# KMASAHIRO/AVR

Hardware: AMD Instinct MI355X
Metric: ray-samples/sec/GPU (1024 rays×256 samp×512 freq) + IR render ms/pose (higher is better)
Workload: dtype f32; 1 GPU; c2_meshrir_1024x256x512; mode=pose, rays=1024, samples=256, T=1022, freq_bins=512, distinct_poses=16, parallelism=poses x1 (no data-path collective)

## Files before the change

### avr_amd/_lib.py

```python
from __future__ import annotations

import ctypes
import math
import os
import threading

import numpy as np
import torch

_HERE = os.path.dirname(os.path.abspath(__file__))
LIB_PATH = os.path.join(_HERE, "libavr_hip.so")

DTYPE_F32 = 0
DTYPE_F16 = 1
DTYPE_BF16 = 2
MAX_AZI = 512
IRFFT_MAX_N = 13476

_c_i32 = ctypes.c_int32
_c_i64 = ctypes.c_int64
_c_f32 = ctypes.c_float
_vp = ctypes.c_void_p


class RenderParams(ctypes.Structure):

    _fields_ = [
        ("n_azi", _c_i32),
        ("n_ele", _c_i32),
        ("n_samples", _c_i32),
        ("T", _c_i32),
        ("n_rays", _c_i32),
        ("depth_scale", _c_f32),
        ("depth_offset", _c_f32),
        ("lo", _c_f32),
        ("span", _c_f32),
        ("fs", _c_f32),
        ("speed", _c_f32),
# ... 22 lines not shown
    p.n_ele = int(cfg["n_ele"])
    p.n_samples = int(cfg["n_samples"])
    p.T = int(T)
    p.n_rays = p.n_azi * p.n_ele + 2 if n_rays is None else int(n_rays)
    p.depth_scale = _f32(cfg["far"] - cfg["near"])
    p.depth_offset = _f32(cfg["near"])
    p.lo = _f32(cfg["xyz_min"])
    p.span = _f32(cfg["xyz_max"] - cfg["xyz_min"])
    p.fs = _f32(cfg["fs"])
    p.speed = _f32(cfg["speed"])
    p.pathloss = _f32(cfg["pathloss"])
    p.azi_jitter = _f32(np.pi * 2 / cfg["n_azi"])
    p.two_pi = _f32(np.pi * 2)
    p.phase_c = _f32((-2 * np.pi) / T)
    p.near_clamp = int(0.1 / cfg["speed"] * cfg["fs"])
    p.pl_len = int(math.ceil(T * 2.5))
    return p


class TablePtrs(ctypes.Structure):

    _fields_ = [("d_vals", ctypes.c_void_p), ("shift", ctypes.c_void_p),
                ("pl_table", ctypes.c_void_p), ("phase", ctypes.c_void_p),
                ("twiddle", ctypes.c_void_p), ("ir_twiddle", ctypes.c_void_p)]


_SIGS = {
    "avr_last_error": (ctypes.c_char_p, []),
    "avr_abi_version": (ctypes.c_int, []),
    "avr_pinned_alloc": (ctypes.c_int, [_c_i64, _vp, _vp]),
    "avr_pinned_free": (ctypes.c_int, [_vp]),
    "avr_graph_launch": (ctypes.c_int, [_vp, _vp]),
    "avr_tables": (ctypes.c_int, [_vp, _vp, _vp, _vp, _vp, _vp, _vp, _vp]),
    "avr_depth_samples": (ctypes.c_int, [_vp, _vp, _vp]),
    "avr_ir_twiddle": (ctypes.c_int, [_c_i32, _vp, _vp]),
    "avr_ray_directions": (ctypes.c_int, [_vp, _vp, _vp, _vp]),
    "avr_sample_points": (ctypes.c_int, [_vp, _c_i32] + [_vp] * 10),
    "avr_sample_rays": (ctypes.c_int, [_vp, _c_i32, _vp, _c_i32] + [_vp] * 9),
    "avr_weights_fwd": (ctypes.c_int, [_vp, _c_i32, _vp, _c_i32] + [_vp] * 7),
    "avr_ray_reduce_fwd": (ctypes.c_int, [_vp, _c_i32, _vp, _c_i32, _vp, _vp, _c_i32, _vp, _vp]),
    "avr_sample_rays_dev": (ctypes.c_int, [_vp, _c_i32, _vp, _c_i32] + [_vp] * 9),
    "avr_sample_rays_staged": (ctypes.c_int, [_vp, _c_i32, _vp, _c_i32, _c_i32] + [_vp] * 7),
    "avr_reduce_splits": (ctypes.c_int, [_vp, _c_i32, _c_i32, _vp]),
    "avr_dft_phase_fwd": (ctypes.c_int, [_vp, _c_i32, _vp, _c_i32, _vp, _vp, _vp, _vp, _c_i32, _vp, _vp]),
    "avr_spectrum_finalize": (ctypes.c_int, [_c_i32, _c_i32, _c_i32, _vp, _vp, _vp]),
    "avr_irfft": (ctypes.c_int, [_c_i32, _c_i32, _vp, _vp, _vp, _vp]),
    "avr_irfft_bwd": (ctypes.c_int, [_c_i32, _c_i32, _vp, _vp, _vp, _vp]),
    "avr_dft_phase_bwd": (ctypes.c_int, [_vp, _c_i32] + [_vp] * 7),
    "avr_ray_reduce_bwd": (ctypes.c_int, [_vp, _c_i32, _vp, _c_i32] + [_vp] * 6),
    "avr_weights_bwd": (ctypes.c_int, [_vp, _c_i32, _vp, _c_i32, _vp, _vp, _vp, _vp]),
    "avr_hashgrid_fwd": (ctypes.c_int, [_c_i64, _c_i32, _vp, _vp, _c_i32, _vp, _vp, _vp, _vp, _c_i32, _vp]),
    "avr_hashgrid_fwd_lm": (ctypes.c_int, [_c_i64, _c_i32, _vp, _vp, _c_i32, _vp, _vp, _vp, _vp, _c_i32, _vp]),
    "avr_hashgrid_fwd_lm_unit": (ctypes.c_int, [_c_i64, _c_i32, _vp, _vp, _c_i32, _vp, _vp, _vp, _vp, _c_i32, _vp]),
    "avr_ray_pose_bias": (ctypes.c_int, [_c_i32, _c_i32, _c_i32, _vp, _vp, _c_i32, _vp, _vp, _vp, _vp,
                                         _c_i32, _vp, _vp, _vp, _vp, _c_i32, _c_i32, _c_i32, _vp, _vp,
                                         _c_i32, _vp, _vp]),
    "avr_hashgrid_bwd": (ctypes.c_int, [_c_i64, _c_i32, _vp, _vp, _c_i32, _vp, _vp, _vp, _vp, _vp]),
    "avr_hashgrid_bwd_workspace": (ctypes.c_int, [_c_i64, _c_i32, _vp, _vp]),
    "avr_hashgrid_bwd_partitioned": (ctypes.c_int, [_c_i64, _c_i32, _vp, _vp, _c_i32, _vp, _vp, _vp, _vp, _vp,
                                                    _c_i64, _vp]),
    "avr_hashgrid_bwd_partitioned_set": (ctypes.c_int, [_c_i64, _c_i32, _vp, _vp, _c_i32, _vp, _vp, _vp, _vp, _vp,
                                                    _c_i64, _vp]),
    "avr_linear_wgrad_splits": (ctypes.c_int, [_c_i64, _c_i32, _c_i32, _vp]),
    "avr_linear512_pack_w2": (ctypes.c_int, [_vp, _c_i32, _c_i32, _vp, _vp]),
    "avr_linear512_mask_fwd": (ctypes.c_int, [_c_i64, _vp, _vp, _c_i32, _vp, _vp, _vp]),
    "avr_linear_wgrad": (ctypes.c_int, [_c_i64, _c_i32, _c_i32, _vp, _vp, _vp, _c_i32, _vp, _vp]),
    "avr_linear_out1_fwd": (ctypes.c_int, [_c_i64, _c_i32, _vp, _vp, _c_i32, _vp, _vp]),
    "avr_narrow_mm": (ctypes.c_int, [_c_i64, _c_i32, _c_i32, _vp, _vp, _c_i32, _c_i32, _vp, _vp, _vp]),
# ... 112 lines not shown
```

### avr_amd/csrc/render_fwd.hip

```cpp
#include "common.h"

#include <cstdlib>

using namespace avr;

typedef float floatx16 __attribute__((ext_vector_type(16)));

namespace {

constexpr double kTwoPi = 6.283185307179586476925286766559;

__global__ void tables_kernel(avr_render_params p, float* __restrict__ d_vals,
                              float* __restrict__ frac, int32_t* __restrict__ shift,
                              float* __restrict__ pl, float2* __restrict__ phase,
                              float2* __restrict__ tw) {
    const int S = p.n_samples, T = p.T, F = T / 2 + 1;
    const int64_t gid = (int64_t)blockIdx.x * blockDim.x + threadIdx.x;
    const int64_t stride = (int64_t)gridDim.x * blockDim.x;
    for (int64_t i = gid; i < S; i += stride) {
        const float d = linspace_at(0.0f, 1.0f, S, (int)i) * p.depth_scale + p.depth_offset;
        const float fr = (p.fs * d) / p.speed;
        d_vals[i] = d;
        frac[i] = fr;
        shift[i] = (int32_t)rintf(fr);
// ... 517 lines not shown
    const float2* src = spart + (int64_t)b * P * F + fc;
    float ax = 0.f, ay = 0.f;
    for (int q0 = 0; q0 < P; q0 += 64) {
        float2 v[4];
#pragma unroll
        for (int u = 0; u < 4; ++u) v[u] = src[(int64_t)min(q0 + g + 16 * u, P - 1) * F];
#pragma unroll
        for (int u = 0; u < 4; ++u)
            if (q0 + g + 16 * u < P) {
                ax += v[u].x;
                ay += v[u].y;
            }
    }
    red[g][j] = make_float2(ax, ay);
    __syncthreads();
    if (g == 0 && f < F) {
        float2 r = red[0][j];
        for (int k = 1; k < 16; ++k) {
            r.x += red[k][j].x;
            r.y += red[k][j].y;
        }
        out[(int64_t)b * F + f] = r;
    }
}

constexpr int kIrfftRedRows = 8;
constexpr size_t irfft_lds(int n) { return (size_t)(n / 2 + 1 + n) * sizeof(float2); }
constexpr size_t irfft_bwd_lds(int n) { return (size_t)n * (sizeof(float2) + sizeof(float)); }
constexpr size_t kIrfftStatic = kIrfftRedRows * 33 * sizeof(float);
constexpr size_t kIrfftBwdStatic = kIrfftRedRows * 33 * sizeof(float2);
static_assert(irfft_lds(kIrfftMaxN) + kIrfftStatic <= kLdsPerCu &&
                  irfft_bwd_lds(kIrfftMaxN) + kIrfftBwdStatic <= kLdsPerCu,
              "AVR_IRFFT_MAX_N must launch in both transforms");
static_assert(kIrfftMaxN % 2 == 0 && irfft_bwd_lds(kIrfftMaxN + 2) + kIrfftBwdStatic > kLdsPerCu,
              "AVR_IRFFT_MAX_N is the largest even length that launches in both");

__global__ __launch_bounds__(256) void irfft_kernel(int F, int B1, const float2* __restrict__ spec,
                                                    const float2* __restrict__ spec2,
                                                    const float2* __restrict__ twg,
                                                    float* __restrict__ ir, float* __restrict__ ir2) {
    extern __shared__ float2 lds[];
    __shared__ float red[kIrfftRedRows][33];
    const int n = 2 * (F - 1);
    float2* X = lds;
    float2* tw = lds + F;
    int b = blockIdx.y;
// ... 349 lines not shown
        return launch("avr_dft_phase_fwd", kern, grid, dim3(kDftThreads), lds, as_stream(stream), *p, part,
                      pl_table, shift, reinterpret_cast<const float2*>(phase),
                      reinterpret_cast<const float2*>(twiddle), reinterpret_cast<float2*>(spart), (int)B, S, T,
                      (int)k_split, kchunk, xcd_order);
    };
    switch (n_split) {
        case 1: return go(dft_phase_fwd_kernel<1>);
        case 2: return go(dft_phase_fwd_kernel<2>);
        case 4: return go(dft_phase_fwd_kernel<4>);
        case 8: return go(dft_phase_fwd_kernel<8>);
        case 16: return go(dft_phase_fwd_kernel<16>);
    }
    return fail(AVR_E_ARG, "avr_dft_phase_fwd: n_split must be 1, 2, 4, 8 or 16");
}

extern "C" int avr_spectrum_finalize(int32_t B, int32_t P, int32_t F, const float* spart,
                                     float* out, void* stream) {
    AVR_REQUIRE(B >= 1 && P >= 1 && F >= 1 && spart && out, "avr_spectrum_finalize: bad args");
    return launch("avr_spectrum_finalize", spectrum_finalize_kernel, dim3((unsigned)((F + 15) / 16), B), dim3(256),
                  0, as_stream(stream), (int)B, (int)P, (int)F, reinterpret_cast<const float2*>(spart),
                  reinterpret_cast<float2*>(out));
}

namespace avr {
int launch_irfft(int B, int F, const float* spec, const float* spec2, const float* tw, float* ir,
                 float* ir2, void* stream) {
    AVR_REQUIRE(B >= 1 && F >= 2 && spec && tw && ir, "avr_irfft: bad args");
    const int n = 2 * (F - 1);
    AVR_REQUIRE(n <= kIrfftMaxN, "avr_irfft: " AVR_IRFFT_LIMIT_TEXT);
    const size_t lds = irfft_lds(n);
    const int rows = spec2 ? 2 * B : B;
    return launch("avr_irfft", irfft_kernel, dim3((n + 31) / 32, rows), dim3(256), lds, as_stream(stream),
                  (int)F, (int)B, reinterpret_cast<const float2*>(spec),
                  reinterpret_cast<const float2*>(spec2 ? spec2 : spec), reinterpret_cast<const float2*>(tw), ir,
                  ir2 ? ir2 : ir);
}
}

extern "C" int avr_irfft(int32_t B, int32_t F, const float* spec, const float* tw, float* ir,
                         void* stream) {
    return avr::launch_irfft(B, F, spec, nullptr, tw, ir, nullptr, stream);
}

extern "C" int avr_irfft_bwd(int32_t B, int32_t F, const float* grad_ir, const float* tw,
                             float* grad_spec, void* stream) {
    AVR_REQUIRE(B >= 1 && F >= 2 && grad_ir && tw && grad_spec, "avr_irfft_bwd: bad args");
// ... 49 lines not shown
    AVR_REQUIRE(B >= 1 && offsets && splits, "avr_render_core_layout: bad args");
    const CoreLayout L = core_layout(p, B, sig_dtype);
    offsets[0] = L.w;
    offsets[1] = L.delay;
    offsets[2] = L.part;
    offsets[3] = L.spart;
    offsets[4] = L.bytes;
    splits[0] = L.n_split;
    splits[1] = L.k_split;
    return 0;
}

extern "C" int avr_render_core_fwd(const avr_render_params* p, int32_t B, const void* attn,
                                   int32_t attn_dtype, const void* signal, int32_t sig_dtype,
                                   const float* rays_o, const float* pos_tx, const float* dirs,
                                   const avr_table_ptrs* tab, void* workspace,
                                   int64_t workspace_bytes, float* out, float* ir, void* ev_begin,
                                   void* ev_end, void* stream) {
    if (int e = validate(p)) return e;
    AVR_REQUIRE(tab && workspace && out, "avr_render_core_fwd: null pointer");
    AVR_REQUIRE(!ir || 2 * (p->T / 2) <= kIrfftMaxN, "avr_render_core_fwd: " AVR_IRFFT_LIMIT_TEXT);
    const CoreLayout L = core_layout(p, B, sig_dtype);
    AVR_REQUIRE(workspace_bytes >= L.bytes, "avr_render_core_fwd: workspace too small");
    char* ws = reinterpret_cast<char*>(workspace);
    float* w = reinterpret_cast<float*>(ws + L.w);
    int32_t* delay = reinterpret_cast<int32_t*>(ws + L.delay);
    float* part = reinterpret_cast<float*>(ws + L.part);
    float* spart = reinterpret_cast<float*>(ws + L.spart);
    if (int e = avr_weights_fwd(p, B, attn, attn_dtype, rays_o, pos_tx, dirs, tab->d_vals, w, delay, stream))
        return e;
    hipStream_t s = as_stream(stream);
    if (ev_begin) (void)hipEventRecord(reinterpret_cast<hipEvent_t>(ev_begin), s);
    if (int e = avr_ray_reduce_fwd(p, B, signal, sig_dtype, w, delay, L.n_split, part, stream))
        return e;
    if (ev_end) (void)hipEventRecord(reinterpret_cast<hipEvent_t>(ev_end), s);
    if (int e = avr_dft_phase_fwd(p, B, part, L.n_split, tab->pl_table, tab->shift, tab->phase, tab->twiddle,
                                  L.k_split, spart, stream))
        return e;
    if (int e = avr_spectrum_finalize(B, L.P, p->T / 2 + 1, spart, out, stream)) return e;
    if (ir) {
        AVR_REQUIRE(tab->ir_twiddle, "avr_render_core_fwd: ir requested without ir_twiddle");
        return avr_irfft(B, p->T / 2 + 1, out, tab->ir_twiddle, ir, stream);
    }
    return 0;
}
```

### avr_amd/renderer.py

```python
from __future__ import annotations

import ctypes
import math
import threading

import torch
import torch.nn as nn

from . import _lib
from ._lib import DTYPE_BF16, DTYPE_F16, DTYPE_F32, _ptr, _stream, render_params
from .options import tuning_env
from .wcache import cache_lookup, cache_store, capturing, cast_weight


_RENDER_KEYS = ("n_samples", "near", "far", "n_azi", "n_ele", "speed", "fs", "pathloss",
                "xyz_min", "xyz_max")


class _NoGuard:
    def __enter__(self):
        return None

    def __exit__(self, *exc):
        return False


_NO_GUARD = _NoGuard()


def _on(dev):
    return _NO_GUARD if torch.cuda.current_device() == dev.index else torch.cuda.device(dev)


def _f32_on(t, dev):
    if t.device != dev or t.dtype != torch.float32:
        t = t.to(dev, torch.float32)
    return t if t.is_contiguous() else t.contiguous()


# ... 10 lines not shown
class Tables:

    def __init__(self, p, device):
        S, T = p.n_samples, p.T
        F = T // 2 + 1
        f32 = dict(dtype=torch.float32, device=device)
        self.d_vals = torch.empty(S, **f32)
        self.frac = torch.empty(S, **f32)
        self.shift = torch.empty(S, dtype=torch.int32, device=device)
        self.pl = torch.empty(p.pl_len, **f32)
        self.phase = torch.empty(S, F, 2, **f32)
        self.twiddle = torch.empty(T, 2, **f32)
        n = 2 * (F - 1)
        self.ir_n = n
        self.ir_twiddle = torch.empty(max(n, 2), 2, **f32)
        st = _stream(device)
        with torch.cuda.device(device):
            _lib.call("avr_tables", ctypes_ref(p), _ptr(self.d_vals), _ptr(self.frac),
                      _ptr(self.shift), _ptr(self.pl), _ptr(self.phase), _ptr(self.twiddle), st)
            if n >= 2:
                _lib.call("avr_ir_twiddle", n, _ptr(self.ir_twiddle), st)
        shifts = self.shift.cpu()
        self.max_shift = int(shifts.max().item()) if S > 0 else 0
        self.ptrs = _lib.TablePtrs(self.d_vals.data_ptr(), self.shift.data_ptr(),
                                   self.pl.data_ptr(), self.phase.data_ptr(),
                                   self.twiddle.data_ptr(),
                                   self.ir_twiddle.data_ptr() if n >= 2 else None)
        self._layouts = {}

    def core_layout(self, p, B, sig_code):
        key = (p.n_rays, B, sig_code) + tuning_env()
        v = self._layouts.get(key)
        if v is None:
            with _TABLE_LOCK:
                v = self._layouts.get(key)
                if v is None:
                    off = (ctypes.c_int64 * 5)()
                    sp = (ctypes.c_int32 * 2)()
                    _lib.call("avr_render_core_layout", ctypes_ref(p), B, sig_code, off, sp)
                    v = (tuple(off), int(sp[0]), int(sp[1]))
                    self._layouts[key] = v
        return v


def ctypes_ref(p):
    return ctypes.byref(p)


_TABLE_CACHE: dict = {}
_TABLE_LOCK = threading.RLock()

# ... 26 lines not shown
    _lib.call("avr_reduce_splits", ctypes_ref(p), B, sig_code, ctypes.byref(n))
    return int(n.value)


def pick_k_split(B, S, T):
    p = _lib.RenderParams(n_azi=1, n_ele=1, n_samples=S, T=T, n_rays=1)
    off = (ctypes.c_int64 * 5)()
    sp = (ctypes.c_int32 * 2)()
    _lib.call("avr_render_core_layout", ctypes_ref(p), B, DTYPE_F32, off, sp)
    return int(sp[1])


def _weights(p, attn, rays_o, position_tx, dirs, tables, st):
    B = attn.size(0)
    R, S = p.n_rays, p.n_samples
    dev = attn.device
    w = torch.empty(B, R, S, dtype=torch.float32, device=dev)
    delay = torch.empty(B, R, S, dtype=torch.int32, device=dev)
    _lib.call("avr_weights_fwd", ctypes_ref(p), B, _ptr(attn), _dtype_code(attn), _ptr(rays_o),
              _ptr(position_tx), _ptr(dirs), _ptr(tables.d_vals), _ptr(w), _ptr(delay), st)
    return w, delay


def _spectrum(p, tables, part, n_split, B, dev, st):
    S, T = p.n_samples, p.T
    F = T // 2 + 1
    k_split = tables.core_layout(p, B, DTYPE_F32)[2]
    P = math.ceil(S / 32) * k_split
    spart = torch.empty(B, P, F, 2, dtype=torch.float32, device=dev)
    _lib.call("avr_dft_phase_fwd", ctypes_ref(p), B, _ptr(part), n_split, _ptr(tables.pl),
              _ptr(tables.shift), _ptr(tables.phase), _ptr(tables.twiddle), k_split,
              _ptr(spart), st)
    out = torch.empty(B, F, 2, dtype=torch.float32, device=dev)
    _lib.call("avr_spectrum_finalize", B, P, F, _ptr(spart), _ptr(out), st)
    return out


def _grad_z(p, tables, grad_out, B, dev, st):
    g = grad_out.contiguous().float()
    gz = torch.empty(B, p.n_samples, p.T, dtype=torch.float32, device=dev)
    _lib.call("avr_dft_phase_bwd", ctypes_ref(p), B, _ptr(g), _ptr(tables.pl), _ptr(tables.shift),
              _ptr(tables.phase), _ptr(tables.twiddle), _ptr(gz), st)
    return gz


def _grad_attn(p, tables, attn, grad_w, st):
    grad_attn = torch.empty_like(attn)
    _lib.call("avr_weights_bwd", ctypes_ref(p), attn.size(0), _ptr(attn), _dtype_code(attn),
              _ptr(tables.d_vals), _ptr(grad_w), _ptr(grad_attn), st)
    return grad_attn


def _render_core_fwd(attn, signal, p, tables, rays_o, position_tx, dirs, ir_out, timer=None):
    dev = signal.device
    B = signal.size(0)
    F = p.T // 2 + 1
    sig_code = _dtype_code(signal)
    off, n_split, _ = tables.core_layout(p, B, sig_code)
    ws = torch.empty(off[4], dtype=torch.uint8, device=dev)
    out = torch.empty(B, F, 2, dtype=torch.float32, device=dev)
    ev0 = ev1 = None
    if timer is not None:
        R, S = p.n_rays, p.n_samples
        delay = ws[off[1]:off[1] + B * R * S * 4].view(torch.int32).view(B, R, S)
        ev0, ev1 = timer.events(n_split=n_split, delay=delay, shift=tables.shift)
    _lib.call("avr_render_core_fwd", ctypes_ref(p), B, _ptr(attn), _dtype_code(attn),
              _ptr(signal), sig_code, _ptr(rays_o), _ptr(position_tx), _ptr(dirs),
              ctypes.byref(tables.ptrs), _ptr(ws), off[4], _ptr(out), _ptr(ir_out), ev0, ev1,
              _stream(dev))
    return out, ws, off


class RenderCore(torch.autograd.Function):

    @staticmethod
    def forward(ctx, attn, signal, p, tables, rays_o, position_tx, dirs, ir_out=None, timer=None):
        out, ws, off = _render_core_fwd(attn, signal, p, tables, rays_o, position_tx, dirs, ir_out, timer)
        B, R, S = signal.size(0), p.n_rays, p.n_samples
        w = ws[off[0]:off[0] + B * R * S * 4].view(torch.float32).view(B, R, S)
        delay = ws[off[1]:off[1] + B * R * S * 4].view(torch.int32).view(B, R, S)
        ctx.p, ctx.tables = p, tables
        ctx.save_for_backward(attn, signal, w, delay)
        return out

    @staticmethod
    def backward(ctx, grad_out):
        attn, signal, w, delay = ctx.saved_tensors
        p, tables = ctx.p, ctx.tables
        dev = signal.device
        B = signal.size(0)
        R, S = p.n_rays, p.n_samples
        st = _stream(dev)
        gz = _grad_z(p, tables, grad_out, B, dev, st)
        grad_signal = torch.empty_like(signal)
        grad_w = torch.empty(B, R, S, dtype=torch.float32, device=dev)
        _lib.call("avr_ray_reduce_bwd", ctypes_ref(p), B, _ptr(signal), _dtype_code(signal),
                  _ptr(gz), _ptr(w), _ptr(delay), _ptr(grad_signal), _ptr(grad_w), st)
        grad_attn = _grad_attn(p, tables, attn, grad_w, st) if ctx.needs_input_grad[0] else None
        return (grad_attn, grad_signal if ctx.needs_input_grad[1] else None,
                None, None, None, None, None, None, None)


def _packed_head_weight(w_master, W, cache, pref, shape_key, st):
    key = (W.data_ptr(), w_master._version, shape_key)
    cache = cache and not capturing()
    if cache:
        hit = cache_lookup(w_master, "_avr_headpack", key)
        if hit is not None:
            return hit
    B, K, code = shape_key[2], shape_key[3], shape_key[4]
    Wp = torch.empty_like(W)
    _lib.call("avr_head_pack_w", pref, B, K, _ptr(W), code, _ptr(Wp), st)
    return cache_store(w_master, "_avr_headpack", key, Wp) if cache else Wp


def _packed_exact_weight(w_master, W, cache, pref, shape_key, nbytes, st):
    key = (W.data_ptr(), w_master._version, shape_key)
    cache = cache and not capturing()
    if cache:
        hit = cache_lookup(w_master, "_avr_exactpack", key)
        if hit is not None:
            return hit
    K, code = shape_key[1], shape_key[2]
    Wf = torch.empty(nbytes // 2, dtype=W.dtype, device=W.device)
    _lib.call("avr_head_pack_w_exact", pref, K, _ptr(W), code, _ptr(Wf), st)
    return cache_store(w_master, "_avr_exactpack", key, Wf) if cache else Wf


class FusedHeadCore(torch.autograd.Function):

    @staticmethod
    def forward(ctx, attn, h, w_master, dtype, p, tables, rays_o, position_tx, dirs, cache=False, exact=False,
                relu_h=False, timer=None):
        dev = h.device
        B, K = h.size(0), h.size(-1)
        S, T = p.n_samples, p.T
        st = _stream(dev)
        pref = ctypes_ref(p)
        W = cast_weight(w_master, dtype, cache)
        code = _dtype_code(h)
        w, delay = _weights(p, attn, rays_o, position_tx, dirs, tables, st)
        R = p.n_rays
        perm = torch.empty(B, S, R, dtype=torch.int32, device=dev)
        ws = torch.empty(B, S, R, dtype=torch.float32, device=dev)
        cnt = torch.empty(B, S, T, dtype=torch.int32, device=dev)
        _lib.call("avr_head_sort", pref, B, _ptr(w), _ptr(delay), _ptr(perm), _ptr(ws), _ptr(cnt), st)
        if exact:
            ns, wbytes = ctypes.c_int32(0), ctypes.c_int64(0)
            _lib.call("avr_head_exact_layout", pref, B, K, code, ctypes.byref(ns), ctypes.byref(wbytes))
            n_split = ns.value
            part = torch.empty(n_split, B, S, T, dtype=torch.float32, device=dev)
            queue = torch.empty(256, dtype=torch.int32, device=dev)
            Wf = _packed_exact_weight(w_master, W, cache, pref, (p.T, K, code), wbytes.value, st)
            ev0, ev1 = timer.head_events(delay, tables.shift, K) if timer is not None else (None, None)
            if ev0 is not None:
                ev0.record()
            _lib.call("avr_head_fwd_exact", pref, B, K, _ptr(h), _ptr(Wf), code, _ptr(perm), _ptr(ws), _ptr(cnt),
                      _ptr(delay), n_split, _ptr(part), _ptr(queue), st)
            if ev1 is not None:
                ev1.record()
        else:
            ns = ctypes.c_int32(0)
            _lib.call("avr_head_splits", pref, B, K, code, ctypes.byref(ns))
            n_split = ns.value
            part = torch.empty(n_split, B, S, T, dtype=torch.float32, device=dev)
            Wp = _packed_head_weight(w_master, W, cache, pref, (p.T, R, B, K, code), st)
            _lib.call("avr_head_fwd", pref, B, K, _ptr(h), _ptr(Wp), code, _ptr(perm), _ptr(ws), _ptr(cnt),
                      n_split, _ptr(part), st)
        out = _spectrum(p, tables, part, n_split, B, dev, st)
        ctx.p, ctx.tables, ctx.relu_h = p, tables, relu_h
        ctx.save_for_backward(attn, h, W, w, delay, perm, ws, cnt)
        return out

    @staticmethod
    def backward(ctx, grad_out):
        attn, h, W, w, delay, perm, ws, cnt = ctx.saved_tensors
        p, tables = ctx.p, ctx.tables
        dev = h.device
        B, K = h.size(0), h.size(-1)
        R, S, T = p.n_rays, p.n_samples, p.T
        st = _stream(dev)
        pref = ctypes_ref(p)
        code = _dtype_code(h)
        gz = _grad_z(p, tables, grad_out, B, dev, st)
        nbytes = ctypes.c_int64(0)
        _lib.call("avr_head_bwd_workspace", pref, B, K, code, ctypes.byref(nbytes))
        work = torch.empty(max(1, nbytes.value // 4), dtype=torch.float32, device=dev)
        grad_h = torch.empty_like(h)
        grad_w = torch.empty(B, R, S, dtype=torch.float32, device=dev)
        grad_W = torch.empty(T, K, dtype=torch.float32, device=dev)
        _lib.call("avr_head_bwd2", pref, B, K, _ptr(h), _ptr(W), code, _ptr(w), _ptr(delay), _ptr(perm),
                  _ptr(ws), _ptr(cnt), _ptr(gz), int(ctx.relu_h), _ptr(grad_h), _ptr(grad_w), _ptr(grad_W),
                  _ptr(work), nbytes.value, st)
        grad_attn = _grad_attn(p, tables, attn, grad_w, st) if ctx.needs_input_grad[0] else None
        return (grad_attn, grad_h if ctx.needs_input_grad[1] else None,
                grad_W if ctx.needs_input_grad[2] else None, None, None, None, None, None, None, None, None, None,
                None)


def _poison_nonfinite(out, tensors, ir_out=None):
    bad = None
    for t in tensors:
        b = ~torch.isfinite(t).all()
        bad = b if bad is None else bad | b
    poison = torch.where(bad, float("nan"), 0.0)
    if ir_out is not None:
        ir_out.add_(poison)
    return out + poison


def normalize_points(input_pts, xyz_min, xyz_max):
    return 2 * (input_pts - xyz_min) / (xyz_max - xyz_min) - 1


def denormalize_points(input_pts, xyz_min, xyz_max):
    return (input_pts + 1) / 2 * (xyz_max - xyz_min) + xyz_min


def draw_jitter(n_azi, n_ele):
    u_azi = torch.rand(n_azi)
# ... 7 lines not shown
    if not random_azi:
        u = torch.zeros_like(u)
    p = render_params(dict(n_azi=n_azi, n_ele=n_ele, n_samples=1, far=1, near=0, xyz_min=-1,
                           xyz_max=1, fs=1, speed=1, pathloss=1), 2)
    dirs = torch.empty(n_azi * n_ele + 2, 3, dtype=torch.float32, device=device)
    u_dev = u.to(device, non_blocking=True)
    _lib.call("avr_ray_directions", ctypes_ref(p), _ptr(u_dev), _ptr(dirs), _stream(device))
    return dirs, None, None


class AVRRender(nn.Module):

    def __init__(self, networks_fn, **kwargs) -> None:
        super().__init__()
        self.network_fn = networks_fn
        for k in _RENDER_KEYS:
            setattr(self, k, kwargs[k])
        self._cfg = {k: kwargs[k] for k in _RENDER_KEYS}
        self.ray_range = None
        self.fused_head = bool(kwargs.get("fused_head", True))
        self.propagate_nonfinite = bool(kwargs.get("propagate_nonfinite", False))
        self.exact_head = bool(kwargs.get("exact_head", True))
        self.head_relu_link = bool(kwargs.get("head_relu_link", True))
        self._pcache = {}
        self._pcache_lock = threading.Lock()
        self._jitter_dev = None
        self._staged = None
        self.kernel_timer = None

    def _device(self, rays_o):
        if rays_o.is_cuda:
            return rays_o.device
        if not torch.cuda.is_available():
            raise RuntimeError("avr_amd.AVRRender needs a HIP device (no CPU fallback)")
        return torch.device("cuda", torch.cuda.current_device())

    def sample(self, rays_o, position_tx, direction_tx=None, u_azi=None):
        if self._staged is not None:
            return self._sample_staged(position_tx.size(0), direction_tx is not None)
        dev = self._device(rays_o)
        B = position_tx.size(0)
        u_dev = self._jitter_dev if u_azi is None else None
        if u_azi is not None and u_azi.is_cuda:
            u_dev, u_azi = u_azi.to(dev, torch.float32).contiguous(), None
        if u_azi is None and u_dev is None:
            u_azi = draw_jitter(self.n_azi, self.n_ele)
# ... 83 lines not shown
        if signal.dtype not in native:
            signal = signal.float()
        if attn.device != dev:
            attn = attn.to(dev)
        attn = attn.reshape(B, -1)
        if not attn.is_contiguous():
            attn = attn.contiguous()
        T = signal.size(-1)
        if signal.device != dev:
            signal = signal.to(dev)
        signal = signal.reshape(B, -1, T)
        if not signal.is_contiguous():
            signal = signal.contiguous()
        R = geom["n_rays"]
        if attn.size(1) != R * S or signal.size(1) != R * S:
            raise ValueError(f"network output has {signal.size(1)} ray-samples, expected "
                             f"{R}x{S}={R * S}")
        p = self._params(T, R)
        with _on(dev):
            tables = get_tables(p, dev)
            check_config(p, tables)
            if not (torch.is_grad_enabled() and (attn.requires_grad or signal.requires_grad)):
                out = _render_core_fwd(attn, signal, p, tables, geom["rays_o"],
                                       geom["position_tx"], geom["dirs"], ir_out, self.kernel_timer)[0]
            else:
                out = RenderCore.apply(attn, signal, p, tables, geom["rays_o"], geom["position_tx"],
                                       geom["dirs"], ir_out, self.kernel_timer)
            if self.propagate_nonfinite:
                out = _poison_nonfinite(out, (attn, signal), ir_out)
            return out

    def _head_supported(self, geom, h, weight, dtype):
        if dtype not in (torch.float32, torch.bfloat16, torch.float16):
            return False
        p = self._params(weight.size(0), geom["n_rays"])
        code = {torch.bfloat16: DTYPE_BF16, torch.float16: DTYPE_F16}.get(dtype, DTYPE_F32)
        n = ctypes.c_int32(0)
        lib = _lib.load()
        if lib.avr_head_splits(ctypes_ref(p), geom["B"], h.size(-1), code, ctypes.byref(n)) != 0:
            return False
        if self._exact_for(dtype, h.size(-1)):
            nb = ctypes.c_int64(0)
            return lib.avr_head_exact_layout(ctypes_ref(p), geom["B"], h.size(-1), code, ctypes.byref(n),
                                             ctypes.byref(nb)) == 0
        return True

    def _exact_for(self, dtype, K):
        return self.exact_head and dtype in (torch.float16, torch.bfloat16) and K % 16 == 0 and K <= 512

    def render_from_hidden(self, attn, h, weight, dtype, geom, relu_link=None):
        dev, B = geom["device"], geom["B"]
        S = int(self.n_samples)
        attn = attn.to(dev).reshape(B, -1)
        if attn.dtype not in (torch.float32, torch.float16, torch.bfloat16):
            attn = attn.float()
        attn = attn.contiguous()
        K, T = h.size(-1), weight.size(0)
        h = h.to(dev, dtype).reshape(B, -1, K).contiguous()
        R = geom["n_rays"]
        if attn.size(1) != R * S or h.size(1) != R * S:
            raise ValueError(f"network output has {h.size(1)} ray-samples, expected {R}x{S}={R * S}")
        p = self._params(T, R)
        with _on(dev):
            tables = get_tables(p, dev)
            check_config(p, tables)
            exact = self._exact_for(dtype, K)
            relu_h = relu_link is not None and torch.is_grad_enabled()
            out = FusedHeadCore.apply(attn, h, weight, dtype, p, tables, geom["rays_o"],
                                      geom["position_tx"], geom["dirs"], not torch.is_grad_enabled(), exact,
                                      relu_h, self.kernel_timer)
            if relu_h:
                relu_link[0] = True
            if self.propagate_nonfinite:
                out = _poison_nonfinite(out, (attn, h, weight))
            return out

    def forward(self, rays_o, position_tx, direction_tx=None, ch_idx=None):
        return self._render(rays_o, position_tx, direction_tx, ch_idx, None)

    def render_ir(self, rays_o, position_tx, direction_tx=None, ch_idx=None):
        ir = []
        grad = torch.is_grad_enabled()
        out = self._render(rays_o, position_tx, direction_tx, ch_idx, None if grad else ir)
        return out, (ir[0] if ir else spectrum_to_ir(out))

    def _render(self, rays_o, position_tx, direction_tx, ch_idx, ir_slot, u_azi=None):
        pts, view, tx, dtx, geom = self.sample(rays_o, position_tx, direction_tx, u_azi=u_azi)
        kw = {} if ch_idx is None else {"ch_idx": ch_idx}
        if getattr(self.network_fn, "accepts_ray_layout", False):
            kw["ray_layout"] = (geom["B"], geom["n_rays"], int(self.n_samples))
        net_in = (pts, view, tx) if dtx is None else (pts, view, tx, dtx)
        if self.fused_head and getattr(self.network_fn, "supports_fused_head", False):
            attn, h, weight, dtype = self.network_fn.forward_fused(*net_in, **kw)
# ... 70 lines not shown
```

### include/avr_hip.h

```cpp
#ifndef AVR_HIP_H
#define AVR_HIP_H

#include <stdint.h>

#ifdef __cplusplus
extern "C" {
#endif

#define AVR_ABI_VERSION 2

#define AVR_DTYPE_F32 0
#define AVR_DTYPE_F16 1
#define AVR_DTYPE_BF16 2

#define AVR_E_ARG 1001
#define AVR_E_CONFIG 1002

typedef struct avr_render_params {
    int32_t n_azi;
    int32_t n_ele;
    int32_t n_samples;
    int32_t T;
    int32_t n_rays;
    float depth_scale;
// ... 45 lines not shown
int avr_sample_rays_staged(const avr_render_params* p, int32_t B, const float* staged,
                           int32_t has_dir_tx, int32_t ray_begin, float* pose_out, float* dirs,
                           float* net_pts, float* net_view, float* net_tx, float* net_dir_tx,
                           void* stream);

int avr_weights_fwd(const avr_render_params* p, int32_t B, const void* attn, int32_t attn_dtype,
                    const float* rays_o, const float* pos_tx, const float* dirs,
                    const float* d_vals, float* w, int32_t* delay, void* stream);

int avr_ray_reduce_fwd(const avr_render_params* p, int32_t B, const void* signal,
                       int32_t sig_dtype, const float* w, const int32_t* delay,
                       int32_t n_split, float* part, void* stream);

int avr_reduce_splits(const avr_render_params* p, int32_t B, int32_t sig_dtype, int32_t* n_split);

int avr_dft_phase_fwd(const avr_render_params* p, int32_t B, const float* part,
                      int32_t n_split, const float* pl_table, const int32_t* shift,
                      const float* phase, const float* twiddle, int32_t k_split,
                      float* spart, void* stream);

int avr_spectrum_finalize(int32_t B, int32_t P, int32_t F, const float* spart, float* out,
                          void* stream);

#define AVR_IRFFT_MAX_N 13476
int avr_irfft(int32_t B, int32_t F, const float* spec, const float* tw, float* ir,
              void* stream);
int avr_irfft_bwd(int32_t B, int32_t F, const float* grad_ir, const float* tw, float* grad_spec,
                  void* stream);

typedef struct avr_table_ptrs {
    const float* d_vals;
    const int32_t* shift;
    const float* pl_table;
    const float* phase;
    const float* twiddle;
    const float* ir_twiddle;
} avr_table_ptrs;

int avr_render_core_layout(const avr_render_params* p, int32_t B, int32_t sig_dtype,
                           int64_t* offsets, int32_t* splits);

int avr_render_core_fwd(const avr_render_params* p, int32_t B, const void* attn,
                        int32_t attn_dtype, const void* signal, int32_t sig_dtype,
                        const float* rays_o, const float* pos_tx, const float* dirs,
                        const avr_table_ptrs* tables, void* workspace, int64_t workspace_bytes,
                        float* out, float* ir, void* ev_begin, void* ev_end, void* stream);

int avr_dft_phase_bwd(const avr_render_params* p, int32_t B, const float* grad_out,
                      const float* pl_table, const int32_t* shift, const float* phase,
                      const float* twiddle, float* gz, void* stream);

int avr_ray_reduce_bwd(const avr_render_params* p, int32_t B, const void* signal,
                       int32_t sig_dtype, const float* gz, const float* w,
                       const int32_t* delay, void* grad_signal, float* grad_w, void* stream);

int avr_weights_bwd(const avr_render_params* p, int32_t B, const void* attn, int32_t attn_dtype,
                    const float* d_vals, const float* grad_w, void* grad_attn, void* stream);

int avr_hashgrid_fwd(int64_t N, int32_t n_levels, const float* x, const void* params,
                     int32_t param_dtype, const int64_t* level_offset, const float* level_scale,
// ... 201 lines not shown
```

Before: 2.300 billion ray-samples/s.

## Replace dense per-sample DFT with Taylor moment expansion of fractional delay phase

Adds a moment-based spectrum transform and makes it the default. The per-sample fractional delay phase is expanded as a 16-term Taylor series, so the time signals are collapsed into 16 moment rows per sample group and only those rows are DFT'd. The aim is to avoid the dense S×T×F phase-weighted DFT. In exchange it adds a truncated-series approximation error and extra workspace, and it changes the ABI struct layout.

```diff
diff --git a/avr_amd/_lib.py b/avr_amd/_lib.py
--- a/avr_amd/_lib.py
+++ b/avr_amd/_lib.py
@@ -14,6 +14,8 @@
 DTYPE_F32 = 0
 DTYPE_F16 = 1
 DTYPE_BF16 = 2
+SPECTRUM_DENSE = 0
+SPECTRUM_MOMENTS = 1
 MAX_AZI = 512
 IRFFT_MAX_N = 13476
 
@@ -82,7 +84,8 @@
 
     _fields_ = [("d_vals", ctypes.c_void_p), ("shift", ctypes.c_void_p),
                 ("pl_table", ctypes.c_void_p), ("phase", ctypes.c_void_p),
-                ("twiddle", ctypes.c_void_p), ("ir_twiddle", ctypes.c_void_p)]
+                ("twiddle", ctypes.c_void_p), ("ir_twiddle", ctypes.c_void_p),
+                ("frac", ctypes.c_void_p), ("spectrum_transform", ctypes.c_int32)]
 
 
 _SIGS = {
@@ -104,6 +107,8 @@
     "avr_reduce_splits": (ctypes.c_int, [_vp, _c_i32, _c_i32, _vp]),
     "avr_dft_phase_fwd": (ctypes.c_int, [_vp, _c_i32, _vp, _c_i32, _vp, _vp, _vp, _vp, _c_i32, _vp, _vp]),
     "avr_spectrum_finalize": (ctypes.c_int, [_c_i32, _c_i32, _c_i32, _vp, _vp, _vp]),
+    "avr_moment_spectrum_workspace": (ctypes.c_int, [_vp, _c_i32, _vp]),
+    "avr_moment_spectrum_fwd": (ctypes.c_int, [_vp, _c_i32, _vp, _c_i32, _vp, _vp, _vp, _vp, _vp, _c_i64, _vp, _vp]),
     "avr_irfft": (ctypes.c_int, [_c_i32, _c_i32, _vp, _vp, _vp, _vp]),
     "avr_irfft_bwd": (ctypes.c_int, [_c_i32, _c_i32, _vp, _vp, _vp, _vp]),
     "avr_dft_phase_bwd": (ctypes.c_int, [_vp, _c_i32] + [_vp] * 7),
diff --git a/avr_amd/csrc/render_fwd.hip b/avr_amd/csrc/render_fwd.hip
--- a/avr_amd/csrc/render_fwd.hip
+++ b/avr_amd/csrc/render_fwd.hip
@@ -563,6 +563,182 @@
         }
         out[(int64_t)b * F + f] = r;
     }
+}
+
+constexpr int kMoments = 16;
+constexpr int kMomThreads = 256;
+constexpr int kMomU = 64;
+constexpr int kMomBatch = 4;
+constexpr int kMomMaxGroups = 16;
+constexpr int kMdftBins = 256;
+
+struct MomentShape {
+    int G, sg;
+    int KS, kchunk;
+};
+
+MomentShape moment_shape(int B, int S, int T) {
+    MomentShape m;
+    const int F = T / 2 + 1;
+    const int nut = (T + kMomU - 1) / kMomU;
+    constexpr int rows = 4 * kMomBatch;
+    int g = (512 + nut * B - 1) / (nut * B);
+    g = max(1, min(g, min(kMomMaxGroups, (S + rows - 1) / rows)));
+    m.sg = ((S + g - 1) / g + rows - 1) / rows * rows;
+    m.G = (S + m.sg - 1) / m.sg;
+    const int nfb = (F + kMdftBins - 1) / kMdftBins, n32 = (T + 31) / 32;
+    int ks = (512 + nfb * B - 1) / (nfb * B);
+    ks = max(1, min(ks, n32));
+    m.kchunk = (n32 + ks - 1) / ks * 32;
+    m.KS = (T + m.kchunk - 1) / m.kchunk;
+    return m;
+}
+
+template <int NS>
+__global__ __launch_bounds__(kMomThreads) void moment_rows_kernel(
+    const float* __restrict__ part, const float* __restrict__ pl, const int32_t* __restrict__ shift,
+    const float* __restrict__ frac, float* __restrict__ mp, int B, int S, int T, int G, int sg) {
+    __shared__ float red[4][kMoments][kMomU];
+    const int g = blockIdx.y, b = blockIdx.z;
+    const int wave = threadIdx.x >> 6, lane = threadIdx.x & 63;
+    const int u = blockIdx.x * kMomU + lane;
+    const int uc = min(u, T - 1);
+    const bool live_u = u < T - 1;
+    const int umax = min((int)blockIdx.x * kMomU + kMomU - 1, T - 2);
+    const int s_begin = g * sg, s_end = min(S, s_begin + sg);
+    const int64_t slab = (int64_t)B * S * T;
+    float acc[kMoments];
+#pragma unroll
+    for (int j = 0; j < kMoments; ++j) acc[j] = 0.0f;
+    for (int s0 = s_begin + wave * kMomBatch; s0 < s_end; s0 += 4 * kMomBatch) {
+        int n[kMomBatch];
+        float dl[kMomBatch];
+        bool row[kMomBatch];
+        bool any = false;
+#pragma unroll
+        for (int i = 0; i < kMomBatch; ++i) {
+            const int sc = min(s0 + i, s_end - 1);
+            n[i] = shift[sc];
+            dl[i] = frac[sc] - (float)n[i];
+            row[i] = s0 + i < s_end && n[i] >= 0 && n[i] <= umax;
+            any |= row[i];
+        }
+        if (!any) continue;
+        float raw[NS][kMomBatch];
+#pragma unroll
+        for (int i = 0; i < kMomBatch; ++i) {
+            const int sc = min(s0 + i, s_end - 1);
+            const int tc = min(max(uc - n[i], 0), T - 1);
+            const int64_t at = ((int64_t)b * S + sc) * T + tc;
+#pragma unroll
+            for (int k = 0; k < NS; ++k) raw[k][i] = part[k * slab + at];
+        }
+#pragma unroll
+        for (int i = 0; i < kMomBatch; ++i) {
+            float sum = raw[0][i];
+#pragma unroll
+            for (int k = 1; k < NS; ++k) sum += raw[k][i];
+            const bool ok = row[i] && live_u && u >= n[i];
+            float v = ok ? sum : 0.0f;
+#pragma unroll
+            for (int j = 0; j < kMoments; ++j) {
+                acc[j] += v;
+                v *= dl[i];
+            }
+        }
+    }
+#pragma unroll
+    for (int j = 0; j < kMoments; ++j) red[wave][j][lane] = acc[j];
+    __syncthreads();
+    if (u < T) {
+        const float gain = live_u ? pl[uc] : 0.0f;
+#pragma unroll
+        for (int i = 0; i < kMoments / 4; ++i) {
+            const int j = wave + 4 * i;
+            const float sum = ((red[0][j][lane] + red[1][j][lane]) + red[2][j][lane]) + red[3][j][lane];
+            mp[(((int64_t)b * G + g) * kMoments + j) * T + u] = live_u ? sum * gain : 0.0f;
+        }
+    }
+}
+
+__constant__ float kInvJ[kMoments] = {
+    0.0f,         1.0f,        1.0f / 2.0f,  1.0f / 3.0f,  1.0f / 4.0f,  1.0f / 5.0f,  1.0f / 6.0f,  1.0f / 7.0f,
+    1.0f / 8.0f,  1.0f / 9.0f, 1.0f / 10.0f, 1.0f / 11.0f, 1.0f / 12.0f, 1.0f / 13.0f, 1.0f / 14.0f, 1.0f / 15.0f};
+
+__global__ __launch_bounds__(kMdftBins) void moment_dft_kernel(const float* __restrict__ mp,
+                                                              const float2* __restrict__ twg,
+                                                              float2* __restrict__ spart, int B, int T, int G,
+                                                              int KS, int kchunk) {
+    extern __shared__ float2 tw[];
+    __shared__ __attribute__((aligned(16))) float As[kMomU][kMoments];
+    const int F = T / 2 + 1;
+    const int ks = blockIdx.y, b = blockIdx.z;
+    const int f = blockIdx.x * kMdftBins + threadIdx.x;
+    const int fm = f < F ? f : 0;
+    const int k0 = ks * kchunk, k1 = min(T, k0 + kchunk);
+    const int col = threadIdx.x & 63, row0 = threadIdx.x >> 6;
+    float re[kMoments], im[kMoments];
+#pragma unroll
+    for (int j = 0; j < kMoments; ++j) {
+        re[j] = 0.0f;
+        im[j] = 0.0f;
+    }
+    float a[kMoments / 4];
+    auto fetch = [&](int kc) {
+#pragma unroll
+        for (int i = 0; i < kMoments / 4; ++i) a[i] = 0.0f;
+        const int uu = min(kc + col, T - 1);
+        for (int g0 = 0; g0 < G; g0 += 4) {
+            float v[4][kMoments / 4];
+#pragma unroll
+            for (int q = 0; q < 4; ++q)
+#pragma unroll
+                for (int i = 0; i < kMoments / 4; ++i)
+                    v[q][i] = mp[(((int64_t)b * G + min(g0 + q, G - 1)) * kMoments + row0 + 4 * i) * T + uu];
+#pragma unroll
+            for (int q = 0; q < 4; ++q)
+#pragma unroll
+                for (int i = 0; i < kMoments / 4; ++i) a[i] += (g0 + q < G) ? v[q][i] : 0.0f;
+        }
+    };
+    if (k0 < k1) fetch(k0);
+    stage_table<kMdftBins>(tw, twg, T);
+    int idx = (int)(((int64_t)k0 * fm) % T);
+    for (int kc = k0; kc < k1; kc += kMomU) {
+        __syncthreads();
+#pragma unroll
+        for (int i = 0; i < kMoments / 4; ++i) As[col][row0 + 4 * i] = (kc + col < k1) ? a[i] : 0.0f;
+        __syncthreads();
+        if (kc + kMomU < k1) fetch(kc + kMomU);
+        const int nu = min(kMomU, k1 - kc);
+        for (int kk = 0; kk < nu; ++kk) {
+            const float2 c = tw[idx];
+            const float4* rowp = reinterpret_cast<const float4*>(As[kk]);
+#pragma unroll
+            for (int q = 0; q < kMoments / 4; ++q) {
+                const float4 m4 = rowp[q];
+                const float mv[4] = {m4.x, m4.y, m4.z, m4.w};
+#pragma unroll
+                for (int e = 0; e < 4; ++e) {
+                    re[4 * q + e] = fmaf(mv[e], c.x, re[4 * q + e]);
+                    im[4 * q + e] = fmaf(mv[e], c.y, im[4 * q + e]);
+                }
+            }
+            idx += fm;
+            if (idx >= T) idx -= T;
+        }
+    }
+    const float th = (float)(kTwoPi * (double)fm / (double)T);
+    float x = re[kMoments - 1], y = im[kMoments - 1];
+#pragma unroll
+    for (int j = kMoments - 1; j >= 1; --j) {
+        const float c = th * kInvJ[j];
+        const float nx = fmaf(c, y, re[j - 1]);
+        const float ny = fmaf(-c, x, im[j - 1]);
+        x = nx;
+        y = ny;
+    }
+    if (f < F) spart[((int64_t)b * KS + ks) * F + f] = make_float2(x, y);
 }
 
 constexpr int kIrfftRedRows = 8;
@@ -958,6 +1134,66 @@
                   reinterpret_cast<float2*>(out));
 }
 
+namespace {
+struct MomentWs {
+    float* mp;
+    float2* spart;
+    int64_t bytes;
+};
+
+MomentWs moment_ws(void* base, const MomentShape& m, int B, int T) {
+    Arena A(base, 256);
+    MomentWs w;
+    w.mp = A.take<float>((int64_t)B * m.G * kMoments * T);
+    w.spart = A.take<float2>((int64_t)B * m.KS * (T / 2 + 1));
+    w.bytes = A.bytes();
+    return w;
+}
+}
+
+extern "C" int avr_moment_spectrum_workspace(const avr_render_params* p, int32_t B, int64_t* bytes) {
+    if (int e = validate(p)) return e;
+    AVR_REQUIRE(B >= 1 && bytes, "avr_moment_spectrum_workspace: bad args");
+    *bytes = moment_ws(nullptr, moment_shape(B, p->n_samples, p->T), B, p->T).bytes;
+    return 0;
+}
+
+extern "C" int avr_moment_spectrum_fwd(const avr_render_params* p, int32_t B, const float* part,
+                                       int32_t n_split, const float* pl_table, const int32_t* shift,
+                                       const float* frac, const float* twiddle, void* workspace,
+                                       int64_t workspace_bytes, float* out, void* stream) {
+    if (int e = validate(p)) return e;
+    AVR_REQUIRE(B >= 1 && part && pl_table && shift && frac && twiddle && workspace && out,
+                "avr_moment_spectrum_fwd: null pointer");
+    const int S = p->n_samples, T = p->T, F = T / 2 + 1;
+    const MomentShape m = moment_shape(B, S, T);
+    const MomentWs w = moment_ws(workspace, m, B, T);
+    AVR_REQUIRE(workspace_bytes >= w.bytes, "avr_moment_spectrum_fwd: workspace too small");
+    const dim3 grid((unsigned)((T + kMomU - 1) / kMomU), (unsigned)m.G, (unsigned)B);
+    auto go = [&](auto kern) {
+        return launch("avr_moment_spectrum_fwd", kern, grid, dim3(kMomThreads), 0, as_stream(stream), part,
+                      pl_table, shift, frac, w.mp, (int)B, S, T, m.G, m.sg);
+    };
+    int e;
+    switch (n_split) {
+        case 1: e = go(moment_rows_kernel<1>); break;
+        case 2: e = go(moment_rows_kernel<2>); break;
+        case 4: e = go(moment_rows_kernel<4>); break;
+        case 8: e = go(moment_rows_kernel<8>); break;
+        case 16: e = go(moment_rows_kernel<16>); break;
+        default: return fail(AVR_E_ARG, "avr_moment_spectrum_fwd: n_split must be 1, 2, 4, 8 or 16");
+    }
+    if (e) return e;
+    float2* dst = m.KS == 1 ? reinterpret_cast<float2*>(out) : w.spart;
+    if (int e2 = launch("avr_moment_spectrum_fwd", moment_dft_kernel,
+                        dim3((unsigned)((F + kMdftBins - 1) / kMdftBins), (unsigned)m.KS, (unsigned)B),
+                        dim3(kMdftBins), (size_t)T * sizeof(float2), as_stream(stream), (const float*)w.mp,
+                        reinterpret_cast<const float2*>(twiddle), dst, (int)B, T, m.G, m.KS, m.kchunk))
+        return e2;
+    if (m.KS == 1) return 0;
+    return avr_spectrum_finalize(B, m.KS, F, reinterpret_cast<const float*>(w.spart), out, stream);
+}
+
 namespace avr {
 int launch_irfft(int B, int F, const float* spec, const float* spec2, const float* tw, float* ir,
                  float* ir2, void* stream) {
@@ -1053,6 +1289,10 @@
     AVR_REQUIRE(!ir || 2 * (p->T / 2) <= kIrfftMaxN, "avr_render_core_fwd: " AVR_IRFFT_LIMIT_TEXT);
     const CoreLayout L = core_layout(p, B, sig_dtype);
     AVR_REQUIRE(workspace_bytes >= L.bytes, "avr_render_core_fwd: workspace too small");
+    const bool moments = tab->spectrum_transform == AVR_SPECTRUM_MOMENTS;
+    AVR_REQUIRE(moments || tab->spectrum_transform == AVR_SPECTRUM_DENSE,
+                "avr_render_core_fwd: unknown spectrum_transform");
+    AVR_REQUIRE(!moments || tab->frac, "avr_render_core_fwd: the moment transform needs tables->frac");
     char* ws = reinterpret_cast<char*>(workspace);
     float* w = reinterpret_cast<float*>(ws + L.w);
     int32_t* delay = reinterpret_cast<int32_t*>(ws + L.delay);
@@ -1065,10 +1305,16 @@
     if (int e = avr_ray_reduce_fwd(p, B, signal, sig_dtype, w, delay, L.n_split, part, stream))
         return e;
     if (ev_end) (void)hipEventRecord(reinterpret_cast<hipEvent_t>(ev_end), s);
-    if (int e = avr_dft_phase_fwd(p, B, part, L.n_split, tab->pl_table, tab->shift, tab->phase, tab->twiddle,
-                                  L.k_split, spart, stream))
-        return e;
-    if (int e = avr_spectrum_finalize(B, L.P, p->T / 2 + 1, spart, out, stream)) return e;
+    if (moments) {
+        if (int e = avr_moment_spectrum_fwd(p, B, part, L.n_split, tab->pl_table, tab->shift, tab->frac,
+                                            tab->twiddle, ws + L.bytes, workspace_bytes - L.bytes, out, stream))
+            return e;
+    } else {
+        if (int e = avr_dft_phase_fwd(p, B, part, L.n_split, tab->pl_table, tab->shift, tab->phase, tab->twiddle,
+                                      L.k_split, spart, stream))
+            return e;
+        if (int e = avr_spectrum_finalize(B, L.P, p->T / 2 + 1, spart, out, stream)) return e;
+    }
     if (ir) {
         AVR_REQUIRE(tab->ir_twiddle, "avr_render_core_fwd: ir requested without ir_twiddle");
         return avr_irfft(B, p->T / 2 + 1, out, tab->ir_twiddle, ir, stream);
diff --git a/avr_amd/renderer.py b/avr_amd/renderer.py
--- a/avr_amd/renderer.py
+++ b/avr_amd/renderer.py
@@ -8,13 +8,15 @@
 import torch.nn as nn
 
 from . import _lib
-from ._lib import DTYPE_BF16, DTYPE_F16, DTYPE_F32, _ptr, _stream, render_params
+from ._lib import (DTYPE_BF16, DTYPE_F16, DTYPE_F32, SPECTRUM_DENSE, SPECTRUM_MOMENTS, _ptr, _stream,
+                   render_params)
 from .options import tuning_env
 from .wcache import cache_lookup, cache_store, capturing, cast_weight
 
 
 _RENDER_KEYS = ("n_samples", "near", "far", "n_azi", "n_ele", "speed", "fs", "pathloss",
                 "xyz_min", "xyz_max")
+SPECTRUM_TRANSFORMS = {"moments": SPECTRUM_MOMENTS, "dense": SPECTRUM_DENSE}
 
 
 class _NoGuard:
@@ -71,11 +73,22 @@
                 _lib.call("avr_ir_twiddle", n, _ptr(self.ir_twiddle), st)
         shifts = self.shift.cpu()
         self.max_shift = int(shifts.max().item()) if S > 0 else 0
-        self.ptrs = _lib.TablePtrs(self.d_vals.data_ptr(), self.shift.data_ptr(),
-                                   self.pl.data_ptr(), self.phase.data_ptr(),
-                                   self.twiddle.data_ptr(),
-                                   self.ir_twiddle.data_ptr() if n >= 2 else None)
+        self.ptrs = {code: _lib.TablePtrs(self.d_vals.data_ptr(), self.shift.data_ptr(),
+                                          self.pl.data_ptr(), self.phase.data_ptr(),
+                                          self.twiddle.data_ptr(),
+                                          self.ir_twiddle.data_ptr() if n >= 2 else None,
+                                          self.frac.data_ptr(), code)
+                     for code in SPECTRUM_TRANSFORMS.values()}
         self._layouts = {}
+        self._moment_ws = {}
+
+    def moment_workspace(self, p, B):
+        v = self._moment_ws.get(B)
+        if v is None:
+            n = ctypes.c_int64(0)
+            _lib.call("avr_moment_spectrum_workspace", ctypes_ref(p), B, ctypes.byref(n))
+            v = self._moment_ws[B] = int(n.value)
+        return v
 
     def core_layout(self, p, B, sig_code):
         key = (p.n_rays, B, sig_code) + tuning_env()
@@ -148,9 +161,16 @@
     return w, delay
 
 
-def _spectrum(p, tables, part, n_split, B, dev, st):
+def _spectrum(p, tables, part, n_split, B, dev, st, transform=SPECTRUM_MOMENTS):
     S, T = p.n_samples, p.T
     F = T // 2 + 1
+    if transform == SPECTRUM_MOMENTS:
+        nbytes = tables.moment_workspace(p, B)
+        ws = torch.empty(nbytes, dtype=torch.uint8, device=dev)
+        out = torch.empty(B, F, 2, dtype=torch.float32, device=dev)
+        _lib.call("avr_moment_spectrum_fwd", ctypes_ref(p), B, _ptr(part), n_split, _ptr(tables.pl),
+                  _ptr(tables.shift), _ptr(tables.frac), _ptr(tables.twiddle), _ptr(ws), nbytes, _ptr(out), st)
+        return out
     k_split = tables.core_layout(p, B, DTYPE_F32)[2]
     P = math.ceil(S / 32) * k_split
     spart = torch.empty(B, P, F, 2, dtype=torch.float32, device=dev)
@@ -177,13 +197,15 @@
     return grad_attn
 
 
-def _render_core_fwd(attn, signal, p, tables, rays_o, position_tx, dirs, ir_out, timer=None):
+def _render_core_fwd(attn, signal, p, tables, rays_o, position_tx, dirs, ir_out, timer=None,
+                     transform=SPECTRUM_MOMENTS):
     dev = signal.device
     B = signal.size(0)
     F = p.T // 2 + 1
     sig_code = _dtype_code(signal)
     off, n_split, _ = tables.core_layout(p, B, sig_code)
-    ws = torch.empty(off[4], dtype=torch.uint8, device=dev)
+    nbytes = off[4] + (tables.moment_workspace(p, B) if transform == SPECTRUM_MOMENTS else 0)
+    ws = torch.empty(nbytes, dtype=torch.uint8, device=dev)
     out = torch.empty(B, F, 2, dtype=torch.float32, device=dev)
     ev0 = ev1 = None
     if timer is not None:
@@ -192,7 +214,7 @@
         ev0, ev1 = timer.events(n_split=n_split, delay=delay, shift=tables.shift)
     _lib.call("avr_render_core_fwd", ctypes_ref(p), B, _ptr(attn), _dtype_code(attn),
               _ptr(signal), sig_code, _ptr(rays_o), _ptr(position_tx), _ptr(dirs),
-              ctypes.byref(tables.ptrs), _ptr(ws), off[4], _ptr(out), _ptr(ir_out), ev0, ev1,
+              ctypes.byref(tables.ptrs[transform]), _ptr(ws), nbytes, _ptr(out), _ptr(ir_out), ev0, ev1,
               _stream(dev))
     return out, ws, off
 
@@ -200,8 +222,10 @@
 class RenderCore(torch.autograd.Function):
 
     @staticmethod
-    def forward(ctx, attn, signal, p, tables, rays_o, position_tx, dirs, ir_out=None, timer=None):
-        out, ws, off = _render_core_fwd(attn, signal, p, tables, rays_o, position_tx, dirs, ir_out, timer)
+    def forward(ctx, attn, signal, p, tables, rays_o, position_tx, dirs, ir_out=None, timer=None,
+                transform=SPECTRUM_MOMENTS):
+        out, ws, off = _render_core_fwd(attn, signal, p, tables, rays_o, position_tx, dirs, ir_out, timer,
+                                        transform)
         B, R, S = signal.size(0), p.n_rays, p.n_samples
         w = ws[off[0]:off[0] + B * R * S * 4].view(torch.float32).view(B, R, S)
         delay = ws[off[1]:off[1] + B * R * S * 4].view(torch.int32).view(B, R, S)
@@ -224,7 +248,7 @@
                   _ptr(gz), _ptr(w), _ptr(delay), _ptr(grad_signal), _ptr(grad_w), st)
         grad_attn = _grad_attn(p, tables, attn, grad_w, st) if ctx.needs_input_grad[0] else None
         return (grad_attn, grad_signal if ctx.needs_input_grad[1] else None,
-                None, None, None, None, None, None, None)
+                None, None, None, None, None, None, None, None)
 
 
 def _packed_head_weight(w_master, W, cache, pref, shape_key, st):
@@ -257,7 +281,7 @@
 
     @staticmethod
     def forward(ctx, attn, h, w_master, dtype, p, tables, rays_o, position_tx, dirs, cache=False, exact=False,
-                relu_h=False, timer=None):
+                relu_h=False, timer=None, transform=SPECTRUM_MOMENTS):
         dev = h.device
         B, K = h.size(0), h.size(-1)
         S, T = p.n_samples, p.T
@@ -293,7 +317,7 @@
             Wp = _packed_head_weight(w_master, W, cache, pref, (p.T, R, B, K, code), st)
             _lib.call("avr_head_fwd", pref, B, K, _ptr(h), _ptr(Wp), code, _ptr(perm), _ptr(ws), _ptr(cnt),
                       n_split, _ptr(part), st)
-        out = _spectrum(p, tables, part, n_split, B, dev, st)
+        out = _spectrum(p, tables, part, n_split, B, dev, st, transform)
         ctx.p, ctx.tables, ctx.relu_h = p, tables, relu_h
         ctx.save_for_backward(attn, h, W, w, delay, perm, ws, cnt)
         return out
@@ -321,7 +345,7 @@
         grad_attn = _grad_attn(p, tables, attn, grad_w, st) if ctx.needs_input_grad[0] else None
         return (grad_attn, grad_h if ctx.needs_input_grad[1] else None,
                 grad_W if ctx.needs_input_grad[2] else None, None, None, None, None, None, None, None, None, None,
-                None)
+                None, None)
 
 
 def _poison_nonfinite(out, tensors, ir_out=None):
@@ -375,6 +399,10 @@
         self.propagate_nonfinite = bool(kwargs.get("propagate_nonfinite", False))
         self.exact_head = bool(kwargs.get("exact_head", True))
         self.head_relu_link = bool(kwargs.get("head_relu_link", True))
+        name = kwargs.get("spectrum_transform", "moments")
+        if name not in SPECTRUM_TRANSFORMS:
+            raise ValueError(f"spectrum_transform must be 'moments' or 'dense', not {name!r}")
+        self.spectrum_transform = name
         self._pcache = {}
         self._pcache_lock = threading.Lock()
         self._jitter_dev = None
@@ -504,10 +532,12 @@
             check_config(p, tables)
             if not (torch.is_grad_enabled() and (attn.requires_grad or signal.requires_grad)):
                 out = _render_core_fwd(attn, signal, p, tables, geom["rays_o"],
-                                       geom["position_tx"], geom["dirs"], ir_out, self.kernel_timer)[0]
+                                       geom["position_tx"], geom["dirs"], ir_out, self.kernel_timer,
+                                       SPECTRUM_TRANSFORMS[self.spectrum_transform])[0]
             else:
                 out = RenderCore.apply(attn, signal, p, tables, geom["rays_o"], geom["position_tx"],
-                                       geom["dirs"], ir_out, self.kernel_timer)
+                                       geom["dirs"], ir_out, self.kernel_timer,
+                                       SPECTRUM_TRANSFORMS[self.spectrum_transform])
             if self.propagate_nonfinite:
                 out = _poison_nonfinite(out, (attn, signal), ir_out)
             return out
@@ -550,7 +580,7 @@
             relu_h = relu_link is not None and torch.is_grad_enabled()
             out = FusedHeadCore.apply(attn, h, weight, dtype, p, tables, geom["rays_o"],
                                       geom["position_tx"], geom["dirs"], not torch.is_grad_enabled(), exact,
-                                      relu_h, self.kernel_timer)
+                                      relu_h, self.kernel_timer, SPECTRUM_TRANSFORMS[self.spectrum_transform])
             if relu_h:
                 relu_link[0] = True
             if self.propagate_nonfinite:
diff --git a/include/avr_hip.h b/include/avr_hip.h
--- a/include/avr_hip.h
+++ b/include/avr_hip.h
@@ -91,6 +91,12 @@
 int avr_spectrum_finalize(int32_t B, int32_t P, int32_t F, const float* spart, float* out,
                           void* stream);
 
+int avr_moment_spectrum_workspace(const avr_render_params* p, int32_t B, int64_t* bytes);
+int avr_moment_spectrum_fwd(const avr_render_params* p, int32_t B, const float* part,
+                            int32_t n_split, const float* pl_table, const int32_t* shift,
+                            const float* frac, const float* twiddle, void* workspace,
+                            int64_t workspace_bytes, float* out, void* stream);
+
 #define AVR_IRFFT_MAX_N 13476
 int avr_irfft(int32_t B, int32_t F, const float* spec, const float* tw, float* ir,
               void* stream);
@@ -104,7 +110,11 @@
     const float* phase;
     const float* twiddle;
     const float* ir_twiddle;
+    const float* frac;
+    int32_t spectrum_transform;
 } avr_table_ptrs;
+#define AVR_SPECTRUM_DENSE 0
+#define AVR_SPECTRUM_MOMENTS 1
 
 int avr_render_core_layout(const avr_render_params* p, int32_t B, int32_t sig_dtype,
                            int64_t* offsets, int32_t* splits);
```

New measurement: 2.303 billion ray-samples/s (median of 6 runs). About the same (+0.1%).
